# noce2/FluidFramework

Hardware: AMD Instinct MI355X
Metric: sequenced merge-tree ops applied/sec (node) at 100k docs; bit-exact text+props (higher is better)
Workload: dtype int32; 1 GPU; c3: 100000 docs/GPU x 10000 sequenced ops, 8 writers, refSeq lag <= 64, insert 0.5 / remove 0.3 / annotate 0.2; docs_total=100000, docs_per_gpu=100000, ops_per_doc=10000, parallelism=doc-shard x1

## Files before the change

fluidframework_amd/__init__.py:

```python
import ctypes

import numpy as np

from . import _native
from .wire import CHECKSUM_DTYPE, OP_DTYPE, Batch, Interner

__all__ = ["MergeTreeBatch", "DeviceBatch", "Batch", "Interner", "DeltaLogOverflow"]


class DeltaLogOverflow(RuntimeError):

    def __init__(self, msg, records):
        super().__init__(msg)
        self.records = records


class PinnedArray:

    def __init__(self, lib, n, dtype):
        dt = np.dtype(dtype)
        nbytes = max(int(n), 1) * dt.itemsize
        self.lib = lib
        self.p = lib.mt_host_alloc(nbytes)
        if not self.p:
            raise MemoryError(f"mt_host_alloc({nbytes}) failed")
        self.a = np.frombuffer((ctypes.c_uint8 * nbytes).from_address(self.p), dtype=dt)

    def __del__(self):
        p, self.p = getattr(self, "p", None), None
        if p:
            try:
                self.lib.mt_host_free(p)
            except Exception:
                pass


class MergeTreeBatch:
# ... 817 lines not shown
                raise ValueError("get_prop_runs_device: out is (runs [rows, 3], records [words])")
        self._check(self.lib.mt_get_prop_runs_bulk_device(*args, ctypes.c_void_p(runs.data_ptr()), runs.shape[0],
                                                          ctypes.c_void_p(recs.data_ptr()), recs.numel()),
                    "mt_get_prop_runs_bulk_device")
        return run_off, word_off, runs[: int(run_off[n])], recs[: int(word_off[n])]

    def last_props_ms(self):
        out = np.zeros(2, dtype=np.float32)
        self._check(self.lib.mt_last_props_ms(self.h, _native.ptr(out)), "mt_last_props_ms")
        return float(out[0]), float(out[1])

    def get_properties_at_position(self, doc, pos):
        return self.get_properties_at_positions([doc], [pos])[0]

    def debug_raw(self, doc):
        n = ctypes.c_uint32()
        hdr = np.zeros(32, dtype=np.int32)
        self._check(self.lib.mt_debug_raw(self.h, doc, None, 0, ctypes.byref(n), _native.ptr(hdr)), "mt_debug_raw")
        rows = np.zeros((max(n.value, 1), 8), dtype=np.uint32)
        self._check(self.lib.mt_debug_raw(self.h, doc, _native.ptr(rows), n.value, ctypes.byref(n), None),
                    "mt_debug_raw")
        return rows[:n.value], hdr

    def is_paged(self, doc):
        return bool(self.debug_raw(doc)[1][24])

    def get_delta_log(self, doc):
        n = ctypes.c_uint32()
        buf = np.zeros(1, dtype=np.int32)
        rc = self.lib.mt_get_delta_log(self.h, doc, None, 0, ctypes.byref(n))
        if rc not in (0, _native.MT_E_OVERFLOW):
            self._check(rc, "mt_get_delta_log")
        buf = np.zeros(max(n.value, 1), dtype=np.int32)
        rc = self.lib.mt_get_delta_log(self.h, doc, _native.ptr(buf), n.value, ctypes.byref(n))
        if rc == _native.MT_E_OVERFLOW:
            raise DeltaLogOverflow(self.lib.mt_last_error(self.h).decode(), buf[: n.value].tolist())
        self._check(rc, "mt_get_delta_log")
        return buf[: n.value].tolist()

    def delta_log_reset(self):
        self._check(self.lib.mt_delta_log_reset(self.h), "mt_delta_log_reset")

    def _dlog_queries(self, docs, from_word):
        if docs is not None:
            docs = np.ascontiguousarray(docs, dtype=np.uint32).reshape(-1)
        n = len(docs) if docs is not None else self.n_docs
# ... 151 lines not shown
```

fluidframework_amd/_native.py:

```python
import ctypes
import os

import numpy as np

from .wire import CHECKSUM_DTYPE, OP_DTYPE

HERE = os.path.dirname(os.path.abspath(__file__))
MT_E_INVALID, MT_E_HIP, MT_E_NOMEM, MT_E_NODEVICE, MT_E_OVERFLOW, MT_E_STALE_VIEW = -1, -2, -3, -4, -5, -6
LIB_PATH = os.environ.get("MT_LIB_PATH") or os.path.join(HERE, "libmtreplay.so")


class MtOptions(ctypes.Structure):
    _fields_ = [("device", ctypes.c_int32), ("seg_capacity", ctypes.c_int32),
                ("block_capacity", ctypes.c_int32), ("heap_capacity", ctypes.c_int32),
                ("text_capacity", ctypes.c_int32), ("props_capacity", ctypes.c_int32),
                ("delta_log_capacity", ctypes.c_int32), ("lds_seg_capacity", ctypes.c_int32),
                ("page_capacity", ctypes.c_int32), ("page_heap_capacity", ctypes.c_int32),
                ("unsettled_capacity", ctypes.c_int32), ("uid_capacity", ctypes.c_int32),
                ("lds_page_capacity", ctypes.c_int32), ("lds_unsettled_capacity", ctypes.c_int32),
                ("lds_page_heap_capacity", ctypes.c_int32), ("lds_narrow_overlap", ctypes.c_int32),
                ("delta_log_mode", ctypes.c_int32), ("live_client", ctypes.c_int32),
                ("live_group_capacity", ctypes.c_int32), ("paged_slices", ctypes.c_int32),
                ("segment_ordinals", ctypes.c_int32), ("overlap_arena_capacity", ctypes.c_int32)]

# ... 93 lines not shown
    ("mt_batch_sizes", _I, [_P, _P, _P, _P]),
    ("mt_batch_download", _I, [_P, _P, _P, _P, _P]),
    ("mt_get_status", _I, [_P, _P]),
    ("mt_get_length", _I, [_P, _U32, _P]),
    ("mt_get_text", _I, [_P, _U32, _P, _U32, _P]),
    ("mt_get_texts", _I, [_P, _U32, _P, _P, _P, ctypes.c_uint16, _P, _P, _U64]),
    ("mt_get_texts_device", _I, [_P, _U32, _P, _P, _P, ctypes.c_uint16, _P, _P, _U64]),
    ("mt_last_text_ms", _I, [_P, _P]),
    ("mt_get_prop_runs", _I, [_P, _U32, _P, _U32, _P, _P, _U32, _P]),
    ("mt_get_prop_runs_bulk", _I, [_P, _U32, _P, _P, _P, _P, _P, _P, _U64, _P, _U64]),
    ("mt_get_prop_runs_bulk_device", _I, [_P, _U32, _P, _P, _P, _P, _P, _P, _U64, _P, _U64]),
    ("mt_last_props_ms", _I, [_P, _P]),
    ("mt_get_segments", _I, [_P, _U32, _P, _U32, _P, _P, _U32, _P]),
    ("mt_get_segment_props", _I, [_P, _U32, _U32, _P, _U32, _P]),
    ("mt_get_all_segment_props", _I, [_P, _U32, _P, ctypes.c_uint64, _P]),
    ("mt_get_overlap_arena", _I, [_P, _U32, _P]),
    ("mt_get_delta_log", _I, [_P, _U32, _P, _U32, _P]),
    ("mt_delta_log_reset", _I, [_P]),
    ("mt_get_delta_logs", _I, [_P, _U32, _P, _P, _P, _P, _P, _P, _U64, _P, _U64]),
    ("mt_get_delta_logs_device", _I, [_P, _U32, _P, _P, _P, _P, _P, _P, _U64, _P, _U64]),
    ("mt_delta_log_reset_docs", _I, [_P, _U32, _P]),
    ("mt_last_dlog_ms", _I, [_P, _P]),
    ("mt_debug_raw", _I, [_P, _U32, _P, _U32, _P, _P]),
    ("mt_debug_pick", _I, [_P, _P, _U32, _P]),
    ("mt_debug_prof", _I, [_P, _P, _I]),
    ("mt_maintenance_counts", _I, [_P, _P]),
    ("mt_checksums", _I, [_P, _P]),
    ("mt_checksums_device", _I, [_P, _P]),
    ("mt_regenerate_pending", _I, [_P, _U32, _P, _U32, _P, _P, _U32, _P, _U32]),
    ("mt_pending_counts", _I, [_P, _P]),
    ("mt_debug_heap", _I, [_P, _U32, _P, _U32, _P, _P, _U32, _P]),
    ("mt_get_containing_segment", _I, [_P, _U32, ctypes.c_int32, ctypes.c_int32, ctypes.c_int32, _P, _P, _U32]),
    ("mt_get_segment_by_uid", _I, [_P, _U32, _U32, ctypes.c_int32, ctypes.c_int32, _P, _P, _U32]),
    ("mt_get_view_lengths", _I, [_P, _U32, _P, _P, _P, _P]),
    ("mt_locate_segments", _I, [_P, _U32, _P, _P, _P, _P, _P]),
    ("mt_locate_uids", _I, [_P, _U32, _P, _P, _P, _P, _P]),
    ("mt_locate_segments_device", _I, [_P, _U32, _P, _P, _P, _P, _P]),
    ("mt_locate_uids_device", _I, [_P, _U32, _P, _P, _P, _P, _P]),
    ("mt_get_view_lengths_bulk", _I, [_P, _U32, _P, _P, _P, _P]),
    ("mt_resolve_remote_positions", _I, [_P, _U32, _P, _P, _P, _P, _P]),
    ("mt_last_locate", _I, [_P, _P, _P]),
    ("mt_find_tiles", _I, [_P, _U32, _P, _P, _P, _P, _U32, _U32, _P, _P, _P]),
    ("mt_find_tiles_device", _I, [_P, _U32, _P, _P, _P, _P, _U32, _U32, _P, _P, _P]),
    ("mt_find_markers_by_id", _I, [_P, _U32, _P, _U32, _P, _P]),
    ("mt_find_markers_by_id_device", _I, [_P, _U32, _P, _U32, _P, _P]),
    ("mt_last_tiles", _I, [_P, _P, _P]),
# ... 36 lines not shown
```

fluidframework_amd/csrc/mt_engine.h:

```cpp
#pragma once
#include <type_traits>

#include "mt_device.h"

#define LDS_AS __attribute__((address_space(3)))
#define GLB_AS __attribute__((address_space(1)))

template <bool kLogT> struct TierLdsT {
    static constexpr bool kLds = true;
    static constexpr bool kLog = kLogT;
    static constexpr bool kPaged = false;
    static constexpr bool kLive = false;
    static constexpr int kOvlBits = 32;
    static constexpr bool kMayGrow = false;
    static constexpr bool kOvf = false;
    typedef uint32_t O_v;
    typedef LDS_AS v4i *A_t;
    typedef LDS_AS uint32_t *O_t;
    typedef LDS_AS v4u *B_t;
    typedef LDS_AS v2i *H_t;
};
template <bool kLogT> struct TierGlbT {
    static constexpr bool kLds = false;
    static constexpr bool kLog = kLogT;
// ... 58 lines not shown
    typedef LDS_AS v4u *B_t;
    typedef LDS_AS v2i *H_t;
};

__device__ __forceinline__ void gsync() { asm volatile("s_waitcnt vmcnt(0)" ::: "memory"); }
__device__ __forceinline__ void gsync_rd() {
#ifdef MT_STRICT_GSYNC
    gsync();
#endif
    __builtin_amdgcn_fence(__ATOMIC_ACQ_REL, "workgroup");
}
template <class T> __device__ __forceinline__ void wsync() {
    if constexpr (T::kLds && !T::kLive)
        asm volatile("" ::: "memory");
    else
        gsync();
}

#define SEGF_NL_KNOWN 1u
#define SEGF_NL 2u
#define SEGF_NOMATCH 4u
#define SEGF_NONL 8u
#define SEGF_SLACK_SHIFT 16
__device__ __forceinline__ int text_slack(int len) { return min((len >> 1) + 8, 4096); }

__device__ static const uint32_t kEmptyPropsRec = 0u;

template <class T> struct DocT {
    DocHdr *hp;
    typename T::A_t A;
    typename T::O_t O;
    typename T::B_t Bv;
    typename T::H_t heap;
    GLB_AS uint16_t *text;
    GLB_AS uint32_t *props;
    GLB_AS int32_t *dlog;
    int32_t S_cap, B_cap, H_cap, T_cap, P_cap, DL_cap;
    LDS_AS uint8_t *cnt;
    LDS_AS int8_t *flg;
    LDS_AS uint16_t *ends;
    LDS_AS int32_t *scr;
    LDS_AS int32_t *nb;
    int n, depth, heap_n, cur_seq, min_seq, text_top, text_half, props_top, props_half, next_uid,
        status, dlog_n, text_gcs, props_gcs, cap_cause;
    u64 dhash;
    int m_split, m_append, m_unlink;
// ... 930 lines not shown
            t[0] = n;
            for (uint32_t k = 0; k < 2 * n; k++) t[1 + k] = s[1 + k];
        }
        wsync<T>();
        if (has) d.Bv[i].y = nh;
        carry += bcast(inc, MT_WAVE - 1);
    }
    d.props_half = dh;
    d.props_top = carry;
    gsync_rd();
    wsync<T>();
}
TD bool props_ensure(DocT<T> &d, int need) {
    if (d.props_top + need <= d.P_cap) return true;
    if constexpr (T::kPaged) {
        if (d.paged) return paged_props_ensure(d, need);
    }
    props_gc(d);
    if (d.status) return false;
    if (d.props_top + need <= d.P_cap) return true;
    fail_cap(d, 5);
    return false;
}
TD bool match_props(DocT<T> &d, uint32_t ha, uint32_t hb, bool nm) {
    if (ha == 0 || hb == 0) return ha == hb;
    if (nm) return false;
    if (ha == hb) return true;
    const GLB_AS uint32_t *a = prec(d, d.props_half, ha), *b = prec(d, d.props_half, hb);
    const uint32_t na = a[0], nbb = b[0];
    if (na != nbb) return false;
    for (uint32_t i = 0; i < na; i++) {
        bool ok = false;
        for (uint32_t j = 0; j < nbb; j++)
            if (b[1 + 2 * j] == a[1 + 2 * i]) ok = b[2 + 2 * j] == a[2 + 2 * i];
        if (!ok) return false;
    }
    return true;
}

struct Cb {
    u64 h;
    int n;
};
TD Cb cb_begin(DocT<T> &d, int seq, int kind) {
    Cb cb;
    cb.h = fnv_u32(fnv_u32(MT_FNV_OFF, (uint32_t)seq), (uint32_t)kind);
    cb.n = 0;
    if constexpr (T::kLog) {
        d.dlog_rec = -1;
        if (d.dlog) {
// ... 324 lines not shown
    v4u b = d.Bv[in ? s + k : s];
    const bool removed = a.z != MT_RSEQ_NONE;
    const bool marker = (b.z & MT_MARKER_BIT) != 0;
    bool pend = false;
    if constexpr (T::kLive) pend = in && pq_any(pq_get(d, in ? s + k : s));
    const bool settled = in && !pend && !removed && a.y <= d.min_seq;
    const bool need_nl = settled && !marker && a.x > 0 && !(b.w & SEGF_NL_KNOWN);
    if (ballot(need_nl)) {
        gsync_rd();
        if (need_nl) {
            const uint16_t ch = text_base(d, d.text_half)[b.x + a.x - 1];
            b.w = (b.w & ~SEGF_NL) | SEGF_NL_KNOWN | (ch == '\n' ? SEGF_NL : 0u);
            d.Bv[s + k].w = b.w;
        }
        wsync<T>();
    }
    const u64 m_unlink = ballot(in && !pend && removed && a.z <= d.min_seq);
    const u64 m_settled = ballot(settled);
    const u64 m_mark = ballot(in && marker);
    const u64 m_nl = ballot(in && (b.w & SEGF_NL) != 0);
    uint32_t owners = 0;
    int prev = -1, plen = 0;
    bool pmark = false, pnl = false, pnm = false;
    uint32_t pprops = 0;
    for (int j = 0; j < cntb; j++) {
        uint32_t own = (uint32_t)j;
        if ((m_unlink >> j) & 1ull) {
            own = 0xF;
            prev = -1;
        } else if (!((m_settled >> j) & 1ull)) {
            prev = -1;
        } else {
            const int lj = bcast(a.x, j);
            const bool mk = (m_mark >> j) & 1ull, nl = (m_nl >> j) & 1ull;
            const uint32_t pj = (uint32_t)bcast((int)b.y, j);
            const bool nmj = (bcast((int)b.w, j) & SEGF_NOMATCH) != 0;
            const bool ok = prev >= 0 && lj > 0 && can_append(plen, pmark, pnl, lj, mk) &&
                            match_props(d, pprops, pj, pnm || nmj);
            if (ok) {
                own = (uint32_t)prev;
                plen += lj;
                pnl = nl;
            } else {
                prev = j;
                plen = lj;
                pmark = mk;
                pnl = !mk && lj > 0 && nl;
                pprops = pj;
                pnm = nmj;
            }
        }
        owners |= own << (4 * j);
    }
    const uint32_t myown = in ? (owners >> (4 * k)) & 0xFu : 0xFu;
    const u64 m_keep = ballot(in && myown == (uint32_t)k);
    const u64 m_app = ballot(in && myown != 0xFu && myown != (uint32_t)k);
    scour_events(d, a, b, m_unlink, m_app, m_keep, s, cntb, 0);
    if (T::kLog) {
        d.m_unlink += __popcll(m_unlink);
        d.m_append += __popcll(m_app);
    }
    if (m_app) {
        mark_dirty(d, s);
        int glen = 0;
        if (in && myown == (uint32_t)k) {
            for (int j = 0; j < cntb; j++) glen += ((owners >> (4 * j)) & 0xFu) == (uint32_t)k ? bcast(a.x, j) : 0;
        }
        u64 m_grp = 0;
        for (int j = 0; j < cntb; j++)
            if ((m_app >> j) & 1ull) m_grp |= 1ull << ((owners >> (4 * j)) & 0xFu);
        int tot = 0;
// ... 53 lines not shown
                    }
                    ntot += lj;
                    np++;
                }
                wsync<T>();
                GLB_AS uint16_t *tb = text_base(d, d.text_half);
                for (int base = 0; base < ntot; base += MT_WAVE) {
                    const int t = base + lane();
                    int src = -1, pre = 0;
                    for (int q = 0; q < np; q++) {
                        const int lq = plen_[q];
                        if (src < 0 && t < pre + lq) src = psrc[q] + (t - pre);
                        pre += lq;
                    }
                    uint16_t ch = 0;
                    if (t < ntot) ch = tb[src];
                    if (t < ntot) tb[dst + t] = ch;
                }
            }
            if (lane() == 0) {
                d.A[s + kk].x = gk;
                v4u nb = bk;
                nb.x = newoff;
                nb.w = (lastw & (SEGF_NL_KNOWN | SEGF_NL)) | nonl | (newslack << SEGF_SLACK_SHIFT);
                d.Bv[s + kk] = nb;
            }
            wsync<T>();
        }
    }
    const int keep = __popcll(m_keep);
    if (keep < cntb) {
        mark_dirty(d, s);
        const bool surv = (m_keep >> k) & 1ull;
        v4i sa;
        u64 so;
        PendQ sp = pq_zero();
        v4u sb;
        uint16_t soc = 0;
        if (surv) {
            sa = d.A[s + k];
            so = d.O[s + k];
            sb = d.Bv[s + k];
            if constexpr (T::kLive) sp = pq_get(d, s + k);
            if (ordon(d)) soc = d.os[s + k];
        }
        const int dst = s + __popcll(m_keep & ((1ull << k) - 1ull));
        wsync<T>();
// ... 15 lines not shown
struct ScourPlan {
    u64 m_join, m_unlink, m_surv;
    bool big;
};
TD ScourPlan scour_plan(DocT<T> &d, const v4i &a, v4u &b, bool in, bool pend, int start, bool &nl_res) {
    const int k = lane();
    const bool removed = a.z != MT_RSEQ_NONE;
    const bool marker = (b.z & MT_MARKER_BIT) != 0;
    const bool cand = in && !pend && !removed && a.y <= d.min_seq;
    nl_res = cand && !marker && a.x > 0 && !(b.w & SEGF_NL_KNOWN);
    if (ballot(nl_res)) {
        P2_T0(9)
        gsync_rd();
        if (nl_res) {
            const uint16_t ch = text_base(d, d.text_half)[b.x + a.x - 1];
            b.w = (b.w & ~SEGF_NL) | SEGF_NL_KNOWN | (ch == '\n' ? SEGF_NL : 0u);
        }
        P2_T1(9)
    }
    const u64 m_cand = ballot(cand);
    const u64 m_mark = ballot(in && marker);
    const u64 m_nl = ballot(in && (b.w & SEGF_NL) != 0);
    const uint32_t pprops = (uint32_t)__shfl_up((int)b.y, 1, MT_WAVE);
    const bool pc = k > 0 && ((m_cand >> (k - 1)) & 1ull);
    const bool pm = k > 0 && ((m_mark >> (k - 1)) & 1ull);
    const bool pn = k > 0 && ((m_nl >> (k - 1)) & 1ull);
#ifdef MT_NO_Q4
    const u64 m_nm = 0;
#else
    const u64 m_nm = ballot(in && (b.w & SEGF_NOMATCH) != 0);
#endif
    const bool nm = ((m_nm >> k) & 1ull) || (k > 0 && ((m_nm >> (k - 1)) & 1ull));
    bool join = cand && pc && k != start && !marker && !pm && !pn && a.x > 0;
    if (join && (nm || pprops != b.y)) join = match_props(d, pprops, b.y, nm);
    ScourPlan p;
    p.m_join = ballot(join);
    p.big = ballot(join && a.x > MT_GRAN) != 0;
    const bool unlink = in && !pend && removed && a.z <= d.min_seq;
    p.m_unlink = ballot(unlink);
    p.m_surv = ballot(in && !unlink && !join);
    return p;
}
struct ScourGroups {
    u64 m_grp;
    int L, gend, glen, totc;
};
__device__ __forceinline__ ScourGroups scour_groups(const v4i &a, bool in, u64 m_join, u64 m_surv) {
    const int k = lane();
    const u64 above = (k < 63) ? (m_join >> (k + 1)) : 0ull;
    ScourGroups g;
    g.m_grp = ballot(((m_surv >> k) & 1ull) && (above & 1ull));
    g.L = g.gend = g.glen = g.totc = 0;
    if (g.m_grp) {
        g.L = wave_scan_incl(in ? a.x : 0);
        g.gend = k + __ffsll((long long)~above) - 1;
        const int Lend = __shfl(g.L, g.gend < MT_WAVE ? g.gend : MT_WAVE - 1, MT_WAVE);
        g.glen = Lend - g.L + (in ? a.x : 0);
// ... 37 lines not shown
            dst = d.text_top + ak;
            move_keeper = true;
            newslack = (uint32_t)text_slack(gk);
            d.text_top += gk + (int)newslack;
        }
        GLB_AS uint16_t *tb = text_base(d, d.text_half);
        const int t0 = move_keeper ? 0 : ak;
        for (int base = t0; base < gk; base += MT_WAVE) {
            const int t = base + lane();
            int src = 0;
            if (t < ak) {
                src = (int)bk.x + t;
            } else {
                for (int j = kk + 1; j <= ge; j++) {
                    const int rj = bcast(Lm, j) - Lk;
                    if (t >= rj) src = bcast((int)bm.x, j) + (t - rj);
                }
            }
            uint16_t ch = 0;
            if (t < gk) ch = tb[src];
            if (t < gk) tb[(move_keeper ? (int)newoff : dst - ak) + t] = ch;
        }
    }
    return ScourKeeper{gk, newoff, (lastw & (SEGF_NL_KNOWN | SEGF_NL)) | nonl | (newslack << SEGF_SLACK_SHIFT)};
}
TD void scour_merge(DocT<T> &d, v4i &a, v4u &b, bool in, const ScourGroups &g) {
    const v4i a0 = a;
    const v4u bm = b;
    for (u64 q = g.m_grp; q; q &= q - 1) {
        const int kk = first_lane(q);
        const v4u bk = v4u{(uint32_t)bcast((int)bm.x, kk), (uint32_t)bcast((int)bm.y, kk),
                           (uint32_t)bcast((int)bm.z, kk), (uint32_t)bcast((int)bm.w, kk)};
        const ScourKeeper r =
            scour_group(d, bk, bcast(a0.x, kk), bm, a0.x, in, g.L, bcast(g.gend, kk), bcast(g.glen, kk), kk);
        if (lane() == kk) {
            a.x = r.len;
            b.x = r.off;
            b.w = r.w;
        }
    }
}


TD int scour_range(DocT<T> &d, int s, int b0, int nbk) {
    int tot = 0;
    for (int q = 0; q < nbk; q++) tot += cntr(d, 0, b0 + q);
    const int k = lane();
// ... 399 lines not shown
        if (cn > MT_KMAX) {
            fail(d, MT_DOC_CAPACITY);
            return;
        }
        if (lane() == 0) {
            GLB_AS uint32_t *t = prec(d, d.props_half, ph);
            uint32_t n = 0;
            for (uint32_t j = 0; j < cntk; j++) {
                if (rec[2 + 2 * j] == MT_VAL_NULL) continue;
                t[1 + 2 * n] = rec[1 + 2 * j];
                t[2 + 2 * n] = rec[2 + 2 * j];
                n++;
            }
            t[0] = n;
        }
#ifndef MT_NO_Q4
        bool nm = false;
        for (uint32_t j = 0; j < cntk; j++) {
            const uint32_t v = rec[2 + 2 * j];
            nm = nm || (v != MT_VAL_NULL && (v & MT_VAL_NOMATCH_BIT));
        }
        if (nm) nomatch = SEGF_NOMATCH;
#endif
    }
    int bstart;
    int B = blk_find(d, 0, ip, false, bstart);
    if (B < 0) {
        FAIL_INTERNAL(d);
        return;
    }
    int bend = bstart + cntr(d, 0, B);
    int x = (js >= 0 && js < bend) ? js : bend;
    if constexpr (T::kLive) {
        while (!d.lop && x == bend) {
            const int s0 = first_v0(d, bend);
            if (s0 < 0 || !is_local_seq(uni(d.A[s0].y)) || B + 1 >= nbr(d, 0)) break;
            B++;
            bstart = bend;
            bend += cntr(d, 0, B);
            x = (js >= 0 && js < bend) ? js : bend;
        }
    }
    uint32_t toff, segw = 0;
    if (marker) {
        toff = op.payload;
    } else {
// ... 89 lines not shown
    for (int q = 0; q < MT_PQ_IDS; q++) {
        const int id = pq_at(pw, q);
        if (id == 0) break;
        const int w1 = d.grp[id * MT_GRP_WORDS + 1];
        if ((w1 & 0xFF) == MT_OP_ANNOTATE && ((w1 >> 8) & 0xFF)) return true;
    }
    return false;
}
TD bool grp_pending_key(DocT<T> &d, const PendQ &pw, uint32_t k) {
    for (int q = 0; q < MT_PQ_IDS; q++) {
        const int id = pq_at(pw, q);
        if (id == 0) break;
        const GLB_AS int32_t *g = d.grp + id * MT_GRP_WORDS;
        if ((g[1] & 0xFF) != MT_OP_ANNOTATE) continue;
        const int nk = (g[1] >> 16) & 0xFF;
        for (int j = 0; j < nk; j++)
            if ((uint32_t)g[2 + j] == k) return true;
    }
    return false;
}

TD bool annotate_record(DocT<T> &d, uint32_t oh, uint32_t nh, const GLB_AS uint32_t *rec, u64 &sh,
                        GLB_AS int32_t *logp, int &nlog, bool *nomatch = nullptr, PendQ pw = pq_zero(),
                        bool *undef = nullptr) {
    const uint32_t cntk = rec[0] & 0xFFFF, comb = rec[0] >> 16;
    const GLB_AS uint32_t *o = oh ? prec(d, d.props_half, oh) : nullptr;
    GLB_AS uint32_t *t = prec(d, d.props_half, nh);
    const uint32_t on = o ? o[0] : 0;
    uint32_t n = 0;
    int npd = 0;
    if constexpr (T::kLive) {
        if (pq_any(pw) && grp_pending_rewrite(d, pw)) {
            for (uint32_t i = 0; i < 2 * on; i++) t[1 + i] = o[1 + i];
            t[0] = on;
            sh = fnv_u32(sh, 0xFFFFFFFFu);
            if (undef) *undef = true;
            return true;
        }
        if (comb == MT_COMBINE_TABLE) pw = pq_zero();
    }
    for (uint32_t i = 0; i < on; i++) {
        const uint32_t k = o[1 + 2 * i], v = o[2 + 2 * i];
        bool in_new = false, truthy = false;
        if constexpr (T::kLive) {
            if (pq_any(pw) && grp_pending_key(d, pw, k)) {
                t[1 + 2 * n] = k;
                t[2 + 2 * n] = v;
                n++;
                continue;
            }
        }
        if (comb == MT_COMBINE_REWRITE) {
            for (uint32_t j = 0; j < cntk; j++)
                if (rec[1 + 2 * j] == k) {
                    in_new = true;
                    const uint32_t nv = rec[2 + 2 * j];
                    truthy = nv != MT_VAL_NULL && !(nv & MT_VAL_FALSY_BIT);
                }
        }
        if (comb == MT_COMBINE_REWRITE && !truthy) {
            const uint32_t dv = in_new ? MT_VAL_NULL : v;
            sh = fnv_u32(fnv_u32(sh, k), dv);
            if (logp) {
                logp[nlog++] = (int32_t)k;
                logp[nlog++] = (int32_t)dv;
            }
            npd++;
        } else {
            t[1 + 2 * n] = k;
            t[2 + 2 * n] = v;
            n++;
        }
    }
    for (uint32_t j = 0; j < cntk; j++) {
        const uint32_t k = rec[1 + 2 * j], v = rec[2 + 2 * j];
        if constexpr (T::kLive) {
            if (pq_any(pw) && grp_pending_key(d, pw, k)) continue;
        }
        int idx = -1;
        for (uint32_t q = 0; q < n; q++)
            if (t[1 + 2 * q] == k) idx = (int)q;
        bool deleted_by_rewrite = false;
        if (comb == MT_COMBINE_REWRITE && idx < 0) {
            for (uint32_t i = 0; i < on; i++)
                if (o[1 + 2 * i] == k) deleted_by_rewrite = true;
        }
        const bool absent = idx < 0 || t[2 + 2 * idx] == MT_VAL_UNDEF;
        if (!deleted_by_rewrite) {
            const uint32_t dv = absent ? MT_VAL_NULL : t[2 + 2 * idx];
            sh = fnv_u32(fnv_u32(sh, k), dv);
            if (logp) {
                logp[nlog++] = (int32_t)k;
                logp[nlog++] = (int32_t)dv;
            }
            npd++;
        }
        uint32_t nv = v;
#ifndef MT_NO_Q4
        if (comb == MT_COMBINE_TABLE) {
            const GLB_AS uint32_t *tab = rec + 1 + 2 * cntk;
            nv = tab[1];
            if (!absent) {
                const uint32_t old = t[2 + 2 * idx];
                bool hit = false;
                for (uint32_t q = 0; q < tab[0]; q++)
                    if (tab[2 + 2 * q] == old) {
                        nv = tab[3 + 2 * q];
                        hit = true;
                    }
                if (!hit) return false;
            }
        }
#endif
        if (nv == MT_VAL_NULL) {
            if (idx >= 0) {
                for (uint32_t q = (uint32_t)idx + 1; q < n; q++) {
                    t[2 * q - 1] = t[2 * q + 1];
                    t[2 * q] = t[2 * q + 2];
                }
                n--;
            }
        } else if (idx >= 0) {
            t[2 + 2 * idx] = nv;
        } else {
            if (n >= MT_KMAX) return false;
            t[1 + 2 * n] = k;
            t[2 + 2 * n] = nv;
            n++;
        }
    }
    t[0] = n;
    sh = fnv_u32(sh, (uint32_t)npd);
    if (nomatch && *nomatch) {
        bool nm = false;
        for (uint32_t q = 0; q < n; q++) nm = nm || (t[2 + 2 * q] & MT_VAL_NOMATCH_BIT) != 0;
        *nomatch = nm;
    }
    return true;
}

TD bool range_mark(DocT<T> &d, const mt_op_rec &op, const GLB_AS uint32_t *rec, int &carry, int &ocarry,
                   Cb &cb) {
    const int r = op.ref_seq, c = op_cli(op), seq = op.seq, p1 = op.pos1, p2 = op.pos2;
    const bool rem = op.kind == MT_OP_REMOVE;
    compute_ends(d);
    if (!rem) gsync_rd();
    int last_b = -1;
    const int L = lane();
    const int nblk = nbr(d, 0);
    bool rec_nm = false;
#ifndef MT_NO_Q4
    if (!rem) {
        rec_nm = (rec[0] >> 16) == MT_COMBINE_TABLE;
        for (uint32_t j = 0; j < (rec[0] & 0xFFFFu); j++) {
// ... 64 lines not shown
        }
        uint32_t nh = 0;
        if (!rem && sel) nh = (uint32_t)(d.props_top + __popcll(sel_m & ((1ull << L) - 1ull)));
        const int ol = v ? obs_len(a) : 0;
        const int oinc = wave_scan_incl(ol);
        const int opos = ocarry + oinc - ol;
        const bool entry = rem ? newly : sel;
        u64 sh = fnv_u32(fnv_u32(MT_FNV_OFF, (uint32_t)opos), (uint32_t)a.x);
        if (!rem && sel) {
            int unused = 0;
            bool nm = rec_nm || (bv.w & SEGF_NOMATCH) != 0;
            PendQ pw = pq_zero();
            if constexpr (T::kLive) {
                PendQ pq = pq_get(d, i);
                if (d.lop) {
                    if (pq_push(pq, d.lg))
                        pq_put(d, i, pq);
                    else
                        bad = true;
                } else {
                    pw = pq;
                }
            }
            if (!annotate_record(d, bv.y, nh, rec, sh, (GLB_AS int32_t *)nullptr, unused, &nm, pw)) bad = true;
            v4u nb = bv;
            nb.y = nh;
            nb.w = (bv.w & ~SEGF_NOMATCH) | (nm ? SEGF_NOMATCH : 0u);
            d.Bv[i] = nb;
        }
        if (ballot(bad)) {
            if (ovl_any && d.ocs == 0 && d.status == 0) d.cap_cause = 11;
            fail(d, MT_DOC_CAPACITY);
            return true;
        }
        if (ballot(spill)) {
            fail_cap(d, 1);
            return true;
        }
        if (!rem) d.props_top += __popcll(sel_m);
        wsync<T>();
        u64 em = ballot(entry);
        while (em) {
            const int j = first_lane(em);
            em &= em - 1;
            cb.h = fnv_u64(cb.h, bcast64(sh, j));
            cb.n++;
            if (T::kLog && d.dlog) {
                cb_log(d, bcast(opos, j));
                cb_log(d, bcast(a.x, j));
                if (!rem) {
// ... 281 lines not shown
```

fluidframework_amd/csrc/mt_paged.h:

```cpp
#pragma once
#include "mt_engine.h"

#ifdef MT_PROF
#define PG_T0(k) const unsigned long long _pt##k = __builtin_amdgcn_s_memtime();
#define PG_T1(k)                                                         \
    if (lane() == 0) {                                                   \
        pd.w.prof[k] += __builtin_amdgcn_s_memtime() - _pt##k;           \
        pd.w.prof[64 + k] += 1ull;                                       \
    }
#define PG_CNT(k)                                                        \
    if (lane() == 0) pd.w.prof[64 + k] += 1ull;
#else
#define PG_T0(k)
#define PG_T1(k)
#define PG_CNT(k)
#endif

template <class T> struct PagedDoc {
    DocT<T> w;
    DocT<T> up;
    LDS_AS PageMeta *meta;
    GLB_AS PageMeta *gmeta;
    LDS_AS int *pvl;
    LDS_AS int *cob;
// ... 1365 lines not shown
    return false;
#else
    return pg_zinplace<T>();
#endif
}
__device__ __forceinline__ int lane_push(int v, int dst) { return __builtin_amdgcn_ds_permute(dst << 2, v); }
TD bool pg_pack_inplace(PagedDoc<T> &pd, int pg, v4i a, v4u b, const ScourPlan &pl, uint32_t bc, int q, int bstart) {
    DocT<T> &w = pd.w;
    const int k = lane();
    const int n = uni(pm_nseg(pd, pg)), nb = uni(pm_nblk(pd, pg));
    const int cnt = pm_bc_of(bc, q);
    const int keep = __popcll(pl.m_surv);
    const int n1 = n - (cnt - keep);
    if (nb > 8) return true;
    const bool in = k >= bstart && k < bstart + cnt;
    const u64 below = (1ull << k) - 1ull;
    const ScourGroups g1 = scour_groups(a, in, pl.m_join, pl.m_surv);
    v4i a1 = a;
    v4u b1 = b;
    if (g1.m_grp) {
        const uint32_t lastw = (uint32_t)__shfl((int)b.w, g1.gend & (MT_WAVE - 1), MT_WAVE);
        if ((g1.m_grp >> k) & 1ull) {
            a1.x = g1.glen;
            b1.w = lastw & (SEGF_NL_KNOWN | SEGF_NL);
        }
    }
    const int d1 = k < bstart ? k
                   : !in      ? k - (cnt - keep)
                   : ((pl.m_surv >> k) & 1ull) ? bstart + __popcll(pl.m_surv & below) : MT_WAVE - 1;
    a1 = v4i{lane_push(a1.x, d1), lane_push(a1.y, d1), lane_push(a1.z, d1), lane_push(a1.w, d1)};
    b1 = v4u{(uint32_t)lane_push((int)b1.x, d1), (uint32_t)lane_push((int)b1.y, d1),
             (uint32_t)lane_push((int)b1.z, d1), (uint32_t)lane_push((int)b1.w, d1)};
    const int src1 = lane_push(k, d1);
    const bool in2 = k < n1;
    int start2 = 0;
    {
        int st = 0;
        for (int j = 0; j < nb; j++) {
            if (k >= st) start2 = st;
            st += j == q ? keep : pm_bc_of(bc, j);
        }
    }
    bool nl2;
    const ScourPlan p2 = scour_plan(w, a1, b1, in2, false, start2, nl2);
    if (p2.big) return true;
    const int total = __popcll(p2.m_surv);
    const PackSplit ps = pack_split(total);
// ... 1431 lines not shown
```

fluidframework_amd/csrc/mt_replay.hip:

```cpp
#include <hip/hip_runtime.h>

#include <algorithm>
#include <cstdlib>
#include <cstdio>
#include <cstring>
#include <map>
#include <mutex>
#include <string>
#include <utility>
#include <vector>

#include "../../include/mt_replay.h"
#include "mt_dlog.h"
#include "mt_kernels.h"
#include "mt_variants.h"
#ifdef MT_SINGLE_TU
#define MT_VARIANT_DEF(n, k, targs) const void *mtk_##n() { return (const void *)(k<MT_UNPAREN targs>); }
MT_VARIANTS(MT_VARIANT_DEF)
#endif

__global__ void __launch_bounds__(MT_WAVE) k_init(DevState st, const int64_t *seed_off,
                                                  const uint16_t *seed) {
    const int doc = blockIdx.x;
    if (doc >= st.n_docs) return;
// ... 33 lines not shown
    int status = !big && (n > st.S || nb0 > st.B) ? MT_DOC_CAPACITY : 0;
    const size_t B = big ? (size_t)nb0 : st.B;
    v4i *dA = big ? sc.A + sc.off[2 * r] : st.segA + doc * (size_t)st.S;
    u64 *dO = big ? sc.O + sc.off[2 * r] : st.segO + doc * (size_t)st.S;
    v4u *dB = big ? sc.B + sc.off[2 * r] : st.segB + doc * (size_t)st.S;
    int ttop = 0, ptop = 1;
    for (int base = 0; base < n && status == 0; base += MT_WAVE) {
        const int i = base + lane();
        const bool v = i < n;
        mt_seg_rec r;
        memset(&r, 0, sizeof(r));
        if (v) r = rs[i];
        const bool marker = (r.flags & MT_F_MARKER) != 0;
        const int tl = v && !marker ? r.len : 0;
        const int hp = v && r.props != MT_NO_PROPS ? 1 : 0;
        const int tinc = wave_scan_incl(tl), pinc = wave_scan_incl(hp);
        const int toff = ttop + tinc - tl, ph = ptop + pinc - hp;
        const int tend = ttop + bcast(tinc, MT_WAVE - 1), pend = ptop + bcast(pinc, MT_WAVE - 1);
        if (tend > st.T || pend > st.P) {
            status = MT_DOC_CAPACITY;
            break;
        }
        bool bad = false, nm = false;
        if (hp) {
            const uint32_t *rec = pin + r.props;
            const uint32_t cnt = rec[0] & 0xFFFF;
            uint32_t *t = props + (size_t)ph * MT_PREC;
            uint32_t k = 0;
            for (uint32_t j = 0; j < cnt; j++) {
                if (rec[2 + 2 * j] == MT_VAL_NULL) continue;
                if (k >= MT_KMAX) {
                    bad = true;
                    break;
                }
                t[1 + 2 * k] = rec[1 + 2 * j];
                t[2 + 2 * k] = rec[2 + 2 * j];
                nm = nm || (rec[2 + 2 * j] & MT_VAL_NOMATCH_BIT) != 0;
                k++;
            }
            t[0] = k;
        }
        if (ballot(bad)) {
            status = MT_DOC_CAPACITY;
            break;
        }
        for (u64 m = ballot(tl > 0); m; m &= m - 1) {
            const int j = first_lane(m);
            const int lj = bcast(tl, j), oj = bcast(toff, j);
            const uint32_t sj = (uint32_t)bcast((int)r.payload, j);
            for (int q = lane(); q < lj; q += MT_WAVE) text[oj + q] = tin[sj + q];
        }
        if (v) {
            const bool rem = r.removed_seq != MT_RSEQ_NONE;
            uint32_t w = 0;
            if (tl > 0) w = SEGF_NL_KNOWN | (tin[r.payload + tl - 1] == '\n' ? SEGF_NL : 0u);
            if (nm) w |= SEGF_NOMATCH;
            dA[i] = v4i{r.len, r.seq, r.removed_seq, pack_cli(r.client, rem ? r.removed_client : 0)};
            dO[i] = 0ull;
            if (st.segP && !big) {
                u64 *w = (u64 *)(st.segP + doc * (size_t)st.S + i);
                w[0] = w[1] = w[2] = w[3] = 0ull;
            }
            dB[i] = v4u{marker ? r.payload : (uint32_t)toff, hp ? (uint32_t)ph : 0u,
                        (uint32_t)(i + 1) | (marker ? MT_MARKER_BIT : 0u), w};
        }
        ttop = tend;
        ptop = pend;
    }
    int nbl[MT_LV];
    int depth = 0, cnt_below = n > 0 ? n : 0, nl = nb0;
    uint8_t *cnt = big ? sc.cnt + MT_LV * sc.off[2 * r + 1] : st.cnt + (size_t)doc * MT_LV * B;
    int8_t *flg = big ? sc.flg + sc.off[2 * r + 1] : st.flg + (size_t)doc * B;
    for (int l = 0; l < MT_LV; l++) nbl[l] = 0;
    while (status == 0) {
        if (depth >= MT_LV) {
            status = MT_DOC_CAPACITY;
            break;
        }
        for (int b = lane(); b < nl; b += MT_WAVE)
// ... 4252 lines not shown
}
int mt_last_tiles(mt_handle *h, int64_t *out, float *ms) {
    if (!h || !out) return MT_E_INVALID;
    out[0] = h->tile_n;
    out[1] = h->tile_rows;
    float t[2] = {0.f, 0.f};
    if (ms) {
        const int rc = read_timer(h, h->tm_tile, t);
        *ms = t[0];
        if (rc) return rc;
    }
    return 0;
}

int mt_debug_raw(mt_handle *h, uint32_t doc, uint32_t *rows, uint32_t cap_rows, uint32_t *n_rows,
                 int32_t *hdr_words) {
    HostDoc hd;
    int rc = fetch_doc(h, doc, hd, false, false);
    if (rc) return rc;
    const int n = hd.hdr.n_seg;
    for (int i = 0; i < n && rows && (uint32_t)i < cap_rows; i++) {
        memcpy(rows + 8 * i, &hd.A[i], 16);
        memcpy(rows + 8 * i + 4, &hd.B[i], 16);
    }
    if (n_rows) *n_rows = (uint32_t)n;
    if (hdr_words) memcpy(hdr_words, &hd.hdr, sizeof(DocHdr));
    return 0;
}

int mt_debug_heap(mt_handle *h, uint32_t doc, int32_t *heap, uint32_t cap, uint32_t *n_heap, int32_t *flags,
                  uint32_t cap_flags, uint32_t *n_flags) {
    HostDoc hd;
    int rc = fetch_doc(h, doc, hd, false, false);
    if (rc) return rc;
    if (hd.hdr.pad[HDR_PAGED]) return MT_E_INVALID;
    const DevState &st = h->st;
    std::vector<int2> hp((size_t)st.H + 1);
    std::vector<int8_t> fl((size_t)st.B);
    HIPCHK(h, hipMemcpy(hp.data(), st.heap + doc * (size_t)(st.H + 1), hp.size() * sizeof(int2), hipMemcpyDeviceToHost));
    HIPCHK(h, hipMemcpy(fl.data(), st.flg + doc * (size_t)st.B, fl.size(), hipMemcpyDeviceToHost));
    const int n = hd.hdr.n_seg;
    for (int k = 1; k <= hd.hdr.heap_n && (uint32_t)(k - 1) < cap; k++) {
        int at = -1;
        for (int i = 0; i < n; i++)
            if ((hd.B[i].z & ~MT_MARKER_BIT) == (uint32_t)hp[k].y) at = i;
        heap[2 * (k - 1)] = hp[k].x;
        heap[2 * (k - 1) + 1] = at;
    }
    if (n_heap) *n_heap = (uint32_t)hd.hdr.heap_n;
    for (int b = 0; b < hd.hdr.n_blk[0] && (uint32_t)b < cap_flags; b++) flags[b] = fl[b];
// ... 380 lines not shown
```

include/mt_replay.h:

```cpp
#ifndef MT_REPLAY_H
#define MT_REPLAY_H
#include <stddef.h>
#include <stdint.h>

#include "mt_types.h"

#ifdef __cplusplus
extern "C" {
#endif

#define MT_E_INVALID (-1)
#define MT_E_HIP (-2)
#define MT_E_NOMEM (-3)
#define MT_E_NODEVICE (-4)
#define MT_E_OVERFLOW (-5)
#define MT_E_STALE_VIEW (-6)

typedef struct mt_handle mt_handle;
typedef struct mt_batch mt_batch;

typedef struct mt_options {
    int32_t device;
    int32_t seg_capacity;
    int32_t block_capacity;
// ... 173 lines not shown
#define MT_WALK_PROPS 2u
typedef struct mt_walk_row {
    int32_t row;
    uint32_t uid;
    int32_t position;
    int32_t length;
    int32_t seq, client;
    int32_t marker_ref_type;
    uint32_t text;
    uint32_t props;
    int32_t start, end;
    uint32_t flags;
} mt_walk_row;
int mt_walk_segments(mt_handle *h, uint32_t n, const uint32_t *docs, const int32_t *start, const int32_t *end,
                     uint32_t what, int64_t *row_off, int64_t *text_off, int64_t *word_off, mt_walk_row *rows,
                     uint64_t cap_rows, uint16_t *text, uint64_t cap_text, uint32_t *records, uint64_t cap_words);
int mt_walk_segments_device(mt_handle *h, uint32_t n, const uint32_t *docs, const int32_t *start, const int32_t *end,
                            uint32_t what, void *row_off_dev, void *text_off_dev, void *word_off_dev, void *rows_dev,
                            uint64_t cap_rows, void *text_dev, uint64_t cap_text, void *records_dev,
                            uint64_t cap_words);
int mt_last_walk_ms(mt_handle *h, float *out );
int mt_debug_raw(mt_handle *h, uint32_t doc, uint32_t *rows, uint32_t cap_rows, uint32_t *n_rows,
                 int32_t *hdr_words);
#define MT_PICK_REPLAY_LDS 0
#define MT_PICK_REPLAY_HBM 1
#define MT_PICK_REPLAY_PAGED 2
#define MT_PICK_GENERATE_LDS 3
#define MT_PICK_GENERATE_HBM 4
#define MT_PICK_GENERATE_PAGED 5
#define MT_PICK_LOAD_CONVERT 6
#define MT_PICK_OCCUPANCY 7
typedef struct mt_pick_query {
    int32_t launch;
    int32_t delta_log, ordinals, live, wpg;
    int32_t big, gen_words;
    int32_t S, B, H;
    int32_t PP, PH, UT, narrow, packed, grow;
} mt_pick_query;
int mt_debug_pick(const mt_pick_query *q, char *name, uint32_t name_cap, uint64_t *lds_bytes);
int mt_debug_prof(mt_handle *h, uint64_t *out , int reset);
int mt_debug_heap(mt_handle *h, uint32_t doc, int32_t *heap, uint32_t cap, uint32_t *n_heap, int32_t *flags,
                  uint32_t cap_flags, uint32_t *n_flags);
int mt_get_delta_log(mt_handle *h, uint32_t doc, int32_t *out, uint32_t cap, uint32_t *n);
int mt_delta_log_reset(mt_handle *h);
#define MT_DLOG_OVERFLOWED 1u
#define MT_DLOG_PAST       2u
// ... 42 lines not shown
```

Before: 170.8 million ops/s.

## Cache a 12-bit property-set signature in segment flags to short-circuit props matching

```diff
diff --git a/fluidframework_amd/__init__.py b/fluidframework_amd/__init__.py
--- a/fluidframework_amd/__init__.py
+++ b/fluidframework_amd/__init__.py
@@ -13,6 +13,11 @@
     def __init__(self, msg, records):
         super().__init__(msg)
         self.records = records
+
+
+def props_signature(pairs):
+    a = np.ascontiguousarray(np.asarray(list(pairs), dtype=np.uint32).reshape(-1, 2))
+    return int(_native.load().mt_props_signature(_native.ptr(a), a.shape[0]))
 
 
 class PinnedArray:
@@ -876,6 +881,14 @@
                     "mt_debug_raw")
         return rows[:n.value], hdr
 
+    def debug_props_sigs(self, doc):
+        n = ctypes.c_uint32()
+        self._check(self.lib.mt_debug_props_sigs(self.h, doc, None, 0, ctypes.byref(n)), "mt_debug_props_sigs")
+        sigs = np.zeros(max(n.value, 1), dtype=np.uint32)
+        self._check(self.lib.mt_debug_props_sigs(self.h, doc, _native.ptr(sigs), n.value, ctypes.byref(n)),
+                    "mt_debug_props_sigs")
+        return sigs[:n.value]
+
     def is_paged(self, doc):
         return bool(self.debug_raw(doc)[1][24])
 
diff --git a/fluidframework_amd/_native.py b/fluidframework_amd/_native.py
--- a/fluidframework_amd/_native.py
+++ b/fluidframework_amd/_native.py
@@ -139,6 +139,8 @@
     ("mt_delta_log_reset_docs", _I, [_P, _U32, _P]),
     ("mt_last_dlog_ms", _I, [_P, _P]),
     ("mt_debug_raw", _I, [_P, _U32, _P, _U32, _P, _P]),
+    ("mt_debug_props_sigs", _I, [_P, _U32, _P, _U32, _P]),
+    ("mt_props_signature", _U32, [_P, _I]),
     ("mt_debug_pick", _I, [_P, _P, _U32, _P]),
     ("mt_debug_prof", _I, [_P, _P, _I]),
     ("mt_maintenance_counts", _I, [_P, _P]),
diff --git a/fluidframework_amd/csrc/mt_engine.h b/fluidframework_amd/csrc/mt_engine.h
--- a/fluidframework_amd/csrc/mt_engine.h
+++ b/fluidframework_amd/csrc/mt_engine.h
@@ -104,6 +104,22 @@
 #define SEGF_NOMATCH 4u
 #define SEGF_NONL 8u
 #define SEGF_SLACK_SHIFT 16
+#define SEGF_PSIG_SHIFT 4
+#define SEGF_PSIG_MASK 0xFFF0u
+__host__ __device__ inline uint32_t mt_psig_mix(uint32_t k, uint32_t v) {
+    uint32_t h = (k * 0x9E3779B1u + v) * 0x85EBCA6Bu;
+    h ^= h >> 15;
+    h *= 0xC2B2AE35u;
+    return (h >> 18) & 0xFFFu;
+}
+__host__ __device__ inline uint32_t psig_put(uint32_t w, uint32_t sig) {
+#ifdef MT_NO_PSIG
+    return w & ~SEGF_PSIG_MASK;
+#else
+    return (w & ~SEGF_PSIG_MASK) | ((sig << SEGF_PSIG_SHIFT) & SEGF_PSIG_MASK);
+#endif
+}
+__host__ __device__ inline uint32_t psig_of(uint32_t w) { return (w & SEGF_PSIG_MASK) >> SEGF_PSIG_SHIFT; }
 __device__ __forceinline__ int text_slack(int len) { return min((len >> 1) + 8, 4096); }
 
 __device__ static const uint32_t kEmptyPropsRec = 0u;
@@ -1080,10 +1096,13 @@
     fail_cap(d, 5);
     return false;
 }
-TD bool match_props(DocT<T> &d, uint32_t ha, uint32_t hb, bool nm) {
+TD bool match_props(DocT<T> &d, uint32_t ha, uint32_t hb, bool nm, uint32_t wa, uint32_t wb) {
     if (ha == 0 || hb == 0) return ha == hb;
     if (nm) return false;
     if (ha == hb) return true;
+#ifndef MT_NO_PSIG
+    if ((wa ^ wb) & SEGF_PSIG_MASK) return false;
+#endif
     const GLB_AS uint32_t *a = prec(d, d.props_half, ha), *b = prec(d, d.props_half, hb);
     const uint32_t na = a[0], nbb = b[0];
     if (na != nbb) return false;
@@ -1454,7 +1473,7 @@
     uint32_t owners = 0;
     int prev = -1, plen = 0;
     bool pmark = false, pnl = false, pnm = false;
-    uint32_t pprops = 0;
+    uint32_t pprops = 0, pw = 0;
     for (int j = 0; j < cntb; j++) {
         uint32_t own = (uint32_t)j;
         if ((m_unlink >> j) & 1ull) {
@@ -1466,9 +1485,10 @@
             const int lj = bcast(a.x, j);
             const bool mk = (m_mark >> j) & 1ull, nl = (m_nl >> j) & 1ull;
             const uint32_t pj = (uint32_t)bcast((int)b.y, j);
-            const bool nmj = (bcast((int)b.w, j) & SEGF_NOMATCH) != 0;
+            const uint32_t wj = (uint32_t)bcast((int)b.w, j);
+            const bool nmj = (wj & SEGF_NOMATCH) != 0;
             const bool ok = prev >= 0 && lj > 0 && can_append(plen, pmark, pnl, lj, mk) &&
-                            match_props(d, pprops, pj, pnm || nmj);
+                            match_props(d, pprops, pj, pnm || nmj, pw, wj);
             if (ok) {
                 own = (uint32_t)prev;
                 plen += lj;
@@ -1479,6 +1499,7 @@
                 pmark = mk;
                 pnl = !mk && lj > 0 && nl;
                 pprops = pj;
+                pw = wj;
                 pnm = nmj;
             }
         }
@@ -1578,7 +1599,8 @@
                 d.A[s + kk].x = gk;
                 v4u nb = bk;
                 nb.x = newoff;
-                nb.w = (lastw & (SEGF_NL_KNOWN | SEGF_NL)) | nonl | (newslack << SEGF_SLACK_SHIFT);
+                nb.w = (lastw & (SEGF_NL_KNOWN | SEGF_NL)) | nonl | (bk.w & SEGF_PSIG_MASK) |
+                       (newslack << SEGF_SLACK_SHIFT);
                 d.Bv[s + kk] = nb;
             }
             wsync<T>();
@@ -1640,6 +1662,11 @@
     const u64 m_mark = ballot(in && marker);
     const u64 m_nl = ballot(in && (b.w & SEGF_NL) != 0);
     const uint32_t pprops = (uint32_t)__shfl_up((int)b.y, 1, MT_WAVE);
+#ifdef MT_NO_PSIG
+    const uint32_t pw = 0;
+#else
+    const uint32_t pw = (uint32_t)__shfl_up((int)b.w, 1, MT_WAVE);
+#endif
     const bool pc = k > 0 && ((m_cand >> (k - 1)) & 1ull);
     const bool pm = k > 0 && ((m_mark >> (k - 1)) & 1ull);
     const bool pn = k > 0 && ((m_nl >> (k - 1)) & 1ull);
@@ -1650,7 +1677,7 @@
 #endif
     const bool nm = ((m_nm >> k) & 1ull) || (k > 0 && ((m_nm >> (k - 1)) & 1ull));
     bool join = cand && pc && k != start && !marker && !pm && !pn && a.x > 0;
-    if (join && (nm || pprops != b.y)) join = match_props(d, pprops, b.y, nm);
+    if (join && (nm || pprops != b.y)) join = match_props(d, pprops, b.y, nm, pw, b.w);
     ScourPlan p;
     p.m_join = ballot(join);
     p.big = ballot(join && a.x > MT_GRAN) != 0;
@@ -1734,7 +1761,9 @@
             if (t < gk) tb[(move_keeper ? (int)newoff : dst - ak) + t] = ch;
         }
     }
-    return ScourKeeper{gk, newoff, (lastw & (SEGF_NL_KNOWN | SEGF_NL)) | nonl | (newslack << SEGF_SLACK_SHIFT)};
+    return ScourKeeper{gk, newoff,
+                       (lastw & (SEGF_NL_KNOWN | SEGF_NL)) | nonl | (bk.w & SEGF_PSIG_MASK) |
+                           (newslack << SEGF_SLACK_SHIFT)};
 }
 TD void scour_merge(DocT<T> &d, v4i &a, v4u &b, bool in, const ScourGroups &g) {
     const v4i a0 = a;
@@ -2180,6 +2209,14 @@
         }
         if (nm) nomatch = SEGF_NOMATCH;
 #endif
+#ifndef MT_NO_PSIG
+        uint32_t sig = 0;
+        for (uint32_t j = 0; j < cntk; j++) {
+            const uint32_t v = rec[2 + 2 * j];
+            if (v != MT_VAL_NULL) sig += mt_psig_mix(rec[1 + 2 * j], v);
+        }
+        nomatch = psig_put(nomatch, sig);
+#endif
     }
     int bstart;
     int B = blk_find(d, 0, ip, false, bstart);
@@ -2315,13 +2352,17 @@
 
 TD bool annotate_record(DocT<T> &d, uint32_t oh, uint32_t nh, const GLB_AS uint32_t *rec, u64 &sh,
                         GLB_AS int32_t *logp, int &nlog, bool *nomatch = nullptr, PendQ pw = pq_zero(),
-                        bool *undef = nullptr) {
+                        bool *undef = nullptr, uint32_t *psig = nullptr) {
     const uint32_t cntk = rec[0] & 0xFFFF, comb = rec[0] >> 16;
     const GLB_AS uint32_t *o = oh ? prec(d, d.props_half, oh) : nullptr;
     GLB_AS uint32_t *t = prec(d, d.props_half, nh);
     const uint32_t on = o ? o[0] : 0;
     uint32_t n = 0;
     int npd = 0;
+    uint32_t sg = 0;
+#ifndef MT_NO_PSIG
+    if (psig) sg = *psig;
+#endif
     if constexpr (T::kLive) {
         if (pq_any(pw) && grp_pending_rewrite(d, pw)) {
             for (uint32_t i = 0; i < 2 * on; i++) t[1 + i] = o[1 + i];
@@ -2359,6 +2400,9 @@
                 logp[nlog++] = (int32_t)dv;
             }
             npd++;
+#ifndef MT_NO_PSIG
+            sg -= mt_psig_mix(k, v);
+#endif
         } else {
             t[1 + 2 * n] = k;
             t[2 + 2 * n] = v;
@@ -2405,6 +2449,10 @@
             }
         }
 #endif
+#ifndef MT_NO_PSIG
+        if (idx >= 0) sg -= mt_psig_mix(k, t[2 + 2 * idx]);
+        if (nv != MT_VAL_NULL) sg += mt_psig_mix(k, nv);
+#endif
         if (nv == MT_VAL_NULL) {
             if (idx >= 0) {
                 for (uint32_t q = (uint32_t)idx + 1; q < n; q++) {
@@ -2423,6 +2471,9 @@
         }
     }
     t[0] = n;
+#ifndef MT_NO_PSIG
+    if (psig) *psig = sg;
+#endif
     sh = fnv_u32(sh, (uint32_t)npd);
     if (nomatch && *nomatch) {
         bool nm = false;
@@ -2533,10 +2584,12 @@
                     pw = pq;
                 }
             }
-            if (!annotate_record(d, bv.y, nh, rec, sh, (GLB_AS int32_t *)nullptr, unused, &nm, pw)) bad = true;
+            uint32_t sg = psig_of(bv.w);
+            if (!annotate_record(d, bv.y, nh, rec, sh, (GLB_AS int32_t *)nullptr, unused, &nm, pw, nullptr, &sg))
+                bad = true;
             v4u nb = bv;
             nb.y = nh;
-            nb.w = (bv.w & ~SEGF_NOMATCH) | (nm ? SEGF_NOMATCH : 0u);
+            nb.w = psig_put((bv.w & ~SEGF_NOMATCH) | (nm ? SEGF_NOMATCH : 0u), sg);
             d.Bv[i] = nb;
         }
         if (ballot(bad)) {
diff --git a/fluidframework_amd/csrc/mt_paged.h b/fluidframework_amd/csrc/mt_paged.h
--- a/fluidframework_amd/csrc/mt_paged.h
+++ b/fluidframework_amd/csrc/mt_paged.h
@@ -1411,7 +1411,7 @@
         const uint32_t lastw = (uint32_t)__shfl((int)b.w, g1.gend & (MT_WAVE - 1), MT_WAVE);
         if ((g1.m_grp >> k) & 1ull) {
             a1.x = g1.glen;
-            b1.w = lastw & (SEGF_NL_KNOWN | SEGF_NL);
+            b1.w = (lastw & (SEGF_NL_KNOWN | SEGF_NL)) | (b.w & SEGF_PSIG_MASK);
         }
     }
     const int d1 = k < bstart ? k
diff --git a/fluidframework_amd/csrc/mt_replay.hip b/fluidframework_amd/csrc/mt_replay.hip
--- a/fluidframework_amd/csrc/mt_replay.hip
+++ b/fluidframework_amd/csrc/mt_replay.hip
@@ -79,6 +79,7 @@
             break;
         }
         bool bad = false, nm = false;
+        uint32_t sig = 0;
         if (hp) {
             const uint32_t *rec = pin + r.props;
             const uint32_t cnt = rec[0] & 0xFFFF;
@@ -93,6 +94,7 @@
                 t[1 + 2 * k] = rec[1 + 2 * j];
                 t[2 + 2 * k] = rec[2 + 2 * j];
                 nm = nm || (rec[2 + 2 * j] & MT_VAL_NOMATCH_BIT) != 0;
+                sig += mt_psig_mix(rec[1 + 2 * j], rec[2 + 2 * j]);
                 k++;
             }
             t[0] = k;
@@ -112,6 +114,7 @@
             uint32_t w = 0;
             if (tl > 0) w = SEGF_NL_KNOWN | (tin[r.payload + tl - 1] == '\n' ? SEGF_NL : 0u);
             if (nm) w |= SEGF_NOMATCH;
+            w = psig_put(w, sig);
             dA[i] = v4i{r.len, r.seq, r.removed_seq, pack_cli(r.client, rem ? r.removed_client : 0)};
             dO[i] = 0ull;
             if (st.segP && !big) {
@@ -4410,10 +4413,27 @@
     for (int i = 0; i < n && rows && (uint32_t)i < cap_rows; i++) {
         memcpy(rows + 8 * i, &hd.A[i], 16);
         memcpy(rows + 8 * i + 4, &hd.B[i], 16);
+        rows[8 * i + 7] &= ~SEGF_PSIG_MASK;
     }
     if (n_rows) *n_rows = (uint32_t)n;
     if (hdr_words) memcpy(hdr_words, &hd.hdr, sizeof(DocHdr));
     return 0;
+}
+
+int mt_debug_props_sigs(mt_handle *h, uint32_t doc, uint32_t *sigs, uint32_t cap_rows, uint32_t *n_rows) {
+    HostDoc hd;
+    int rc = fetch_doc(h, doc, hd, false, false);
+    if (rc) return rc;
+    const int n = hd.hdr.n_seg;
+    for (int i = 0; i < n && sigs && (uint32_t)i < cap_rows; i++) sigs[i] = psig_of(hd.B[i].w);
+    if (n_rows) *n_rows = (uint32_t)n;
+    return 0;
+}
+
+uint32_t mt_props_signature(const uint32_t *pairs, int n) {
+    uint32_t sig = 0;
+    for (int j = 0; j < n; j++) sig += mt_psig_mix(pairs[2 * j], pairs[2 * j + 1]);
+    return sig & 0xFFFu;
 }
 
 int mt_debug_heap(mt_handle *h, uint32_t doc, int32_t *heap, uint32_t cap, uint32_t *n_heap, int32_t *flags,
diff --git a/include/mt_replay.h b/include/mt_replay.h
--- a/include/mt_replay.h
+++ b/include/mt_replay.h
@@ -219,6 +219,8 @@
 int mt_last_walk_ms(mt_handle *h, float *out );
 int mt_debug_raw(mt_handle *h, uint32_t doc, uint32_t *rows, uint32_t cap_rows, uint32_t *n_rows,
                  int32_t *hdr_words);
+uint32_t mt_props_signature(const uint32_t *pairs, int n);
+int mt_debug_props_sigs(mt_handle *h, uint32_t doc, uint32_t *sigs, uint32_t cap_rows, uint32_t *n_rows);
 #define MT_PICK_REPLAY_LDS 0
 #define MT_PICK_REPLAY_HBM 1
 #define MT_PICK_REPLAY_PAGED 2
```

After: 176.0 million ops/s (median of 6 runs). 1.03x the previous value.
